# alexnodeland/fugue

Measured on AMD Instinct MI355X. Metric: hmc_leapfrog_steps_per_sec, higher is better.
Workload: dtype f64; 1 GPU; C2-normal32: hmc_chain, 32-site conjugate Normal (x#i~N(0,1), y#i~N(x#i,0.5)=0.2i-1), 65536 chains/GPU, L=16, HMCConfig::default; chains_per_gpu=65536, chains_total=65536, n_leapfrog=16, transitions_per_launch=25

## Files before the change

fugue_amd/csrc/fg_hmc_sep.hip:

```cpp
#include "fg_engine_internal.h"
#include "fg_gradstream.h"
#define FG_COLD_UKEY 1
#include "fg_cold.h"
#include "fg_hmc_sep_plan.h"

static_assert(FG_SEP_WAVE == FG_WAVE, "fg_hmc_sep_plan.h sizes tiles for 64-lane waves");

struct FgSepArgs {
    FgProgramDev P; FgChainCtx X; FgHmcDev H; FgSegSep seg;
    int iter0, n_steps, n_warmup, welford_on;
    double *draws; int first_sample_t;
    double *pos_all, *info;
};
static_assert(alignof(FgProgramDev) == 8 && alignof(FgChainCtx) == 8 && alignof(FgHmcDev) == 8 && alignof(FgSegSep) == 4, "kernarg layout of k_hmc_sep_steps");
static_assert(offsetof(FgSepArgs, X) == sizeof(FgProgramDev) && offsetof(FgSepArgs, H) == offsetof(FgSepArgs, X) + sizeof(FgChainCtx) &&
              offsetof(FgSepArgs, seg) == offsetof(FgSepArgs, H) + sizeof(FgHmcDev) && offsetof(FgSepArgs, iter0) == offsetof(FgSepArgs, seg) + sizeof(FgSegSep) &&
              offsetof(FgSepArgs, welford_on) == offsetof(FgSepArgs, iter0) + 12 && offsetof(FgSepArgs, draws) == ((offsetof(FgSepArgs, welford_on) + 4 + 7) & ~(size_t)7) &&
              offsetof(FgSepArgs, first_sample_t) == offsetof(FgSepArgs, draws) + 8 && offsetof(FgSepArgs, pos_all) == offsetof(FgSepArgs, draws) + 16 &&
              offsetof(FgSepArgs, info) == offsetof(FgSepArgs, draws) + 24, "kernarg layout of k_hmc_sep_steps: every argument at the next multiple of its alignment");

#ifdef FG_HMC_PROF
__device__ unsigned long long fg_hmc_prof[FG_SEP_WMAX][8];
#define FG_PROF_T(i) { const unsigned long long now_ = __builtin_readcyclecounter(); prof_[i] += now_ - tprev_; tprev_ = now_; }
#else
#define FG_PROF_T(i)
#endif
#ifndef FG_SEP_STAGGER
#define FG_SEP_STAGGER 2
#endif

__device__ __forceinline__ fg_u32x8 fg_sep_ld8(const FG_AS4 char *p) { return *(const FG_AS4 fg_u32x8 *)p; }
__device__ __forceinline__ fg_u32x4 fg_sep_ld4(const FG_AS4 char *p) { return *(const FG_AS4 fg_u32x4 *)p; }
__device__ __forceinline__ fg_u32x8 fg_sep_ld8(const char *p) { return *(const fg_u32x8 *)p; }
__device__ __forceinline__ fg_u32x4 fg_sep_ld4(const char *p) { return *(const fg_u32x4 *)p; }
__device__ __forceinline__ const FG_AS4 FgSepArgs *fg_sep_kernargs() {
    const FG_AS4 FgSepArgs *ka = (const FG_AS4 FgSepArgs *)__builtin_amdgcn_kernarg_segment_ptr();
    asm volatile("" : "+s"(ka));
    return ka;
}
__device__ __forceinline__ int fg_sep_scalar(int v) { asm volatile("" : "+s"(v)); return v; }
#define FG_SEP_LOAD(k) \
    const fg_u32x8 a##k = fg_sep_ld8(rb + 64 * k); \
    const fg_u32x4 b##k = fg_sep_ld4(rb + 64 * k + 32);

#define FG_SEP_Z(k, dl) (P2 ? (dl) * fg_dbl(a##k[4], a##k[5])                                                                   \
                            : ((a##k[0] & FG_G_POW2) ? (dl) * fg_dbl(a##k[4], a##k[5])                                           \
                                                     : ((a##k[0] & FG_G_DIV) ? (dl) / fg_dbl(b##k[0], b##k[1])                    \
                                                                             : fg_div_const((dl), fg_dbl(b##k[0], b##k[1]), fg_dbl(a##k[4], a##k[5])))))
#define FG_SEP_LP(k, z) (-0.5 * (z) * (z) - fg_dbl(a##k[6], a##k[7]) - 0.5 * FG_LN_2PI)
#define FG_SEP_DUAL(k, outp, outm)                                                                     \
    double outp, outm;                                                                                 \
    { const double c = fg_dbl(a##k[2], a##k[3]); const double zp = FG_SEP_Z(k, qp - c), zm = FG_SEP_Z(k, qm - c); \
      outp = FG_SEP_LP(k, zp); outm = FG_SEP_LP(k, zm); }
#define FG_SEP_NAN_NEG_INF(z, lp) { if (__builtin_expect(__any((z) != (z)), 0)) lp = ((z) != (z)) ? FG_NEG_INF : lp; }
#define FG_SEP_TERM_TO(k, dst)                                                                         \
    { const double z = FG_SEP_Z(k, q - fg_dbl(a##k[2], a##k[3])); double lp = FG_SEP_LP(k, z);       \
      FG_SEP_NAN_NEG_INF(z, lp) (dst)[a##k[1] * tw] = lp; }
#define FG_SEP_TERM(k) FG_SEP_TERM_TO(k, terms)
#define FG_SEP_LP_U(z) (-0.5 * (z) * (z) - 0.5 * FG_LN_2PI)
#define FG_SEP_LPF(k, z) (__builtin_fma(-0.5, (z) * (z), -fg_dbl(a##k[6], a##k[7])) - 0.5 * FG_LN_2PI)
#define FG_SEP_LPF_U(z) __builtin_fma(-0.5, (z) * (z), -0.5 * FG_LN_2PI)
#define FG_SEP_DUALF(k, outp, outm)                                                                    \
    double outp, outm;                                                                                 \
    { const double c = fg_dbl(a##k[2], a##k[3]); const double zp = FG_SEP_Z(k, qp - c), zm = FG_SEP_Z(k, qm - c); \
      outp = FG_SEP_LPF(k, zp); outm = FG_SEP_LPF(k, zm); }
#define FG_SEP_DUALS(k, outp, outm)                                                                    \
    double outp, outm;                                                                                 \
    { const double c = fg_dbl(a##k[2], a##k[3]); const double dp = qp - c, dm = qm - c;                \
      outp = __builtin_fma(nhs2_##k, dp * dp, -fg_dbl(a##k[6], a##k[7])) - 0.5 * FG_LN_2PI;            \
      outm = __builtin_fma(nhs2_##k, dm * dm, -fg_dbl(a##k[6], a##k[7])) - 0.5 * FG_LN_2PI; }
#define FG_SEPD_OWN(k, outp, outm) double outp, outm;                                                  \
    { const double c_ = fg_dbl(a##k[2], a##k[3]); const double zp_ = FG_SEP_Z(k, qp - c_), zm_ = FG_SEP_Z(k, qm - c_); \
      const double lp_ = FG_SEP_LP(k, zp_), lm_ = FG_SEP_LP(k, zm_);                                    \
      outp = (zp_ != zp_) ? FG_NEG_INF : lp_; outm = (zm_ != zm_) ? FG_NEG_INF : lm_; }

template <typename RB> struct FgSepScalarRb { static constexpr bool value = false; };
template <> struct FgSepScalarRb<const FG_AS4 char *> { static constexpr bool value = true; };

template <int NOBS, bool P2, bool CHECK, bool AN = false, bool U0 = false, bool FOLD = false, typename RB = const FG_AS4 char *, bool RANGED = false>
__device__ __forceinline__ bool fg_sep_trajectory(RB rb, double &q_io, double &p_io, double emi, double hk, int L, double h, double two_h,
                                                  double rcp_2h, double *terms, int tw, int nobs_rt, double c_hi = 0.0, double c_lo = 0.0) {
#define FG_SEP_HAS(k) (NOBS >= 0 ? NOBS >= (k) : nobs_rt >= (k))
    FG_SEP_LOAD(0) FG_SEP_LOAD(1) FG_SEP_LOAD(2) FG_SEP_LOAD(3)
    double q = q_io, p = p_io;
    bool bad = false;
    constexpr bool FOLDED = FOLD && P2 && !CHECK && !AN;
    double nhs2_0 = 0.0, nhs2_1 = 0.0, nhs2_2 = 0.0, nhs2_3 = 0.0;
#define FG_SEP_NHS2(k) if (FOLDED && (k > 0 || !U0) && FG_SEP_HAS(k)) { nhs2_##k = fg_dbl(b##k[2], b##k[3]); asm volatile("" : "+v"(nhs2_##k)); }
    FG_SEP_NHS2(0) FG_SEP_NHS2(1) FG_SEP_NHS2(2) FG_SEP_NHS2(3)
#undef FG_SEP_NHS2
    if (FOLD && !CHECK && !AN && FgSepScalarRb<RB>::value) asm volatile("" : "+s"(h), "+s"(c_hi), "+s"(c_lo));
    if (CHECK && !AN && NOBS >= 0 && FgSepScalarRb<RB>::value) asm volatile("" : "+s"(h));
    uint32_t nrange = 0u;
    auto grad = [&]() __attribute__((always_inline)) -> double {
        double g;
        if (AN) {
#define FG_SEP_ANTERM(k) { const double dl = q - fg_dbl(a##k[2], a##k[3]);                                                   \
        const double w = (P2 || (a##k[0] & FG_G_POW2)) ? (dl * fg_dbl(a##k[4], a##k[5])) * fg_dbl(a##k[4], a##k[5])         \
                                                       : (dl / fg_dbl(b##k[0], b##k[1])) / fg_dbl(b##k[0], b##k[1]); g = g - w; }
            g = 0.0;
            FG_SEP_ANTERM(0)
            if (FG_SEP_HAS(1)) FG_SEP_ANTERM(1)
            if (FG_SEP_HAS(2)) FG_SEP_ANTERM(2)
            if (FG_SEP_HAS(3)) FG_SEP_ANTERM(3)
#undef FG_SEP_ANTERM
        } else {
        const double qp = q + h, qm = q - h;
        double tp, tm;
        if (FOLDED) {
            if (U0) { tp = FG_SEP_LPF_U(qp); tm = FG_SEP_LPF_U(qm); }
            else { FG_SEP_DUALS(0, tp_, tm_) tp = tp_; tm = tm_; }
            if (FG_SEP_HAS(1)) {
                FG_SEP_DUALS(1, lp1, lm1)
                double sp = lp1, sm = lm1;
                if (FG_SEP_HAS(2)) { FG_SEP_DUALS(2, lp2, lm2) sp += lp2; sm += lm2; }
                if (FG_SEP_HAS(3)) { FG_SEP_DUALS(3, lp3, lm3) sp += lp3; sm += lm3; }
                tp = tp + sp; tm = tm + sm;
            }
        } else if (!CHECK) {
            if (U0) { tp = FG_SEP_LPF_U(qp); tm = FG_SEP_LPF_U(qm); }
            else { FG_SEP_DUALF(0, tp_, tm_) tp = tp_; tm = tm_; }
            if (FG_SEP_HAS(1)) {
                FG_SEP_DUALF(1, lp1, lm1)
                double sp = lp1, sm = lm1;
                if (FG_SEP_HAS(2)) { FG_SEP_DUALF(2, lp2, lm2) sp += lp2; sm += lm2; }
                if (FG_SEP_HAS(3)) { FG_SEP_DUALF(3, lp3, lm3) sp += lp3; sm += lm3; }
                tp = tp + sp; tm = tm + sm;
            }
        } else {
        if (U0) { tp = FG_SEP_LP_U(qp); tm = FG_SEP_LP_U(qm); }
        else { FG_SEP_DUAL(0, tp_, tm_) tp = tp_; tm = tm_; }
        if (FG_SEP_HAS(1)) {
            FG_SEP_DUAL(1, lp1, lm1)
            double sp = lp1, sm = lm1;
            if (FG_SEP_HAS(2)) { FG_SEP_DUAL(2, lp2, lm2) sp += lp2; sm += lm2; }
            if (FG_SEP_HAS(3)) { FG_SEP_DUAL(3, lp3, lm3) sp += lp3; sm += lm3; }
            tp = tp + sp; tm = tm + sm;
        }
        }
        const double n = tp - tm;
        if (!CHECK && FOLD) g = __builtin_fma(n, c_hi, n * c_lo);
        else g = fg_div_const(n, two_h, rcp_2h);
        if (!CHECK && FOLD && RANGED) {
        } else if (!CHECK && FOLD) {
            uint32_t hi = (uint32_t)__double2hiint(n);
            asm("" : "+v"(hi));
            const uint32_t nr = (hi << 1) - 0x19000000u;
            nrange = nrange > nr ? nrange : nr;
        } else {
        const double an = __builtin_fabs(n);
        if (__builtin_expect(__any(!(an >= 0x1p-823 && an <= 0x1p953)), 0)) g = n / two_h;
        }
        }
        if (CHECK) bad = bad || !fg_finite(g);
        return g;
    };
    { const double kick = hk * grad(); p = p + kick; asm volatile(""); q = q + emi * p; }
    for (int gs = 1; gs < L; ++gs) {
        const double kick = hk * grad();
        p = p + kick;
        asm volatile(""); p = p + kick;
        asm volatile(""); q = q + emi * p;
    }
    { const double kick = hk * grad(); p = p + kick; }
    if (!CHECK && FOLD && !RANGED && nrange >= 0xde000000u) p = __builtin_nan("");
    if (U0) { double lp = FG_SEP_LP_U(q); FG_SEP_NAN_NEG_INF(q, lp) terms[a0[1] * tw] = lp; }
    else FG_SEP_TERM(0)
    if (FG_SEP_HAS(1)) FG_SEP_TERM(1)
    if (FG_SEP_HAS(2)) FG_SEP_TERM(2)
    if (FG_SEP_HAS(3)) FG_SEP_TERM(3)
    q_io = q; p_io = p;
    return bad;
#undef FG_SEP_HAS
}

template <bool AN, typename RB>
__device__ __noinline__ FgD3 fg_sep_trajectory_checked(RB rb, double q, double p, double emi, double hk, int L, double h,
                                                       double two_h, double rcp_2h, double *terms, int tw, int nobs) {
    const bool bad = fg_sep_trajectory<-1, false, true, AN, false, false, RB>(rb, q, p, emi, hk, L, h, two_h, rcp_2h, terms, tw, nobs);
    FgD3 r; r.a = q; r.b = p; r.c = bad ? 1.0 : 0.0;
    return r;
}

template <int K, bool PSON>
__device__ __forceinline__ void fg_dense_add_rows(const double *p, int cnt, int tw, double &PS, double (&ap)[4], double (&am)[4]) {
#define FG_DENSE_BLOCK(R) { double y[R];                                                        \
        _Pragma("unroll") for (int q = 0; q < R; ++q) y[q] = p[q * tw];                         \
        _Pragma("unroll") for (int q = 0; q < R; ++q) { if (PSON) PS += y[q];                   \
            _Pragma("unroll") for (int jj = 0; jj < K; ++jj) { ap[jj] += y[q]; am[jj] += y[q]; } } \
        p += (long long)R * tw; }
    for (; cnt >= 8; cnt -= 8) FG_DENSE_BLOCK(8)
    if (cnt & 4) FG_DENSE_BLOCK(4)
    if (cnt & 2) FG_DENSE_BLOCK(2)
    if (cnt & 1) FG_DENSE_BLOCK(1)
#undef FG_DENSE_BLOCK
}
template <int NC>
__device__ __forceinline__ void fg_dense_section(const double *T, int tw, int lo, int hi, const int (&r)[4], const double (&tp)[4], const double (&tm)[4],
                                                 double (&ap)[4], double (&am)[4]) {
    double PS = 0.0;
    int pos = lo;
#define FG_DENSE_STEP(J) if (NC > J) {                                                          \
        fg_dense_add_rows<J, true>(T + (long long)pos * tw, r[J] - pos, tw, PS, ap, am);       \
        const double x = T[(long long)r[J] * tw];                                               \
        ap[J] = PS + tp[J]; am[J] = PS + tm[J];                                                 \
        _Pragma("unroll") for (int jj = 0; jj < J; ++jj) { ap[jj] += x; am[jj] += x; }          \
        if (NC > J + 1) PS += x;                                                                \
        pos = r[J] + 1; }
    FG_DENSE_STEP(0) FG_DENSE_STEP(1) FG_DENSE_STEP(2) FG_DENSE_STEP(3)
#undef FG_DENSE_STEP
    fg_dense_add_rows<NC, false>(T + (long long)pos * tw, hi - pos, tw, PS, ap, am);
}

template <int NC, bool OBS, bool MASS>
__device__ __forceinline__ bool fg_dense_trajectory(const FgProgramDev &P, const FgChainCtx &X, const FgHmcDev &H, const int (&own)[4], double *T0, double *T1,
                                                    double *kin0, double *kin1, int tw, int n_pri, int n_s, int L, double e, double h, double two_h,
                                                    double rcp_2h, uint32_t sk0, uint32_t sk1, uint32_t gchain, uint32_t iter, long long c, bool live) {
    int ci[4] = {0, 0, 0, 0}, rP[4] = {0, 0, 0, 0}, rO[4] = {0, 0, 0, 0};
    double q[4], p[4], k0v[4], mii[4], cP[4], sP[4], lP[4], cO[4], sO[4], lO[4];
    const double hk = 0.5 * e;
    const int blk_a = own[0] >> 1;
    int blk_b = blk_a;
#pragma unroll
    for (int j = 1; j < NC; ++j) if ((own[j] >> 1) != blk_a) blk_b = own[j] >> 1;
    const FgD2 za = fg_cold_normal_pair(sk0, sk1, gchain, (uint32_t)blk_a, iter, FG_RNG_HMC);
    FgD2 zb2 = za;
    if (NC > 2) zb2 = fg_cold_normal_pair(sk0, sk1, gchain, (uint32_t)blk_b, iter, FG_RNG_HMC);
#pragma unroll
    for (int j = 0; j < NC; ++j) {
        ci[j] = own[j];
        const FgSepCoord cd = P.sep_coord[ci[j]];
        const FG_AS4 char *rb = (const FG_AS4 char *)(uintptr_t)(P.sep + cd.off);
        { FG_SEP_LOAD(0) rP[j] = (int)a0[1]; cP[j] = fg_dbl(a0[2], a0[3]); sP[j] = fg_dbl(a0[4], a0[5]); lP[j] = fg_dbl(a0[6], a0[7]); (void)b0; }
        if (OBS) { FG_SEP_LOAD(1) rO[j] = (int)a1[1]; cO[j] = fg_dbl(a1[2], a1[3]); sO[j] = fg_dbl(a1[4], a1[5]); lO[j] = fg_dbl(a1[6], a1[7]); (void)b1; }
        const bool in_a = (ci[j] >> 1) == blk_a, second = (ci[j] & 1) != 0;
        const double z = in_a ? (second ? za.b : za.a) : (second ? zb2.b : zb2.a);
        mii[j] = MASS ? H.m_inv[(long long)ci[j] * X.C + c] : 1.0;
        p[j] = MASS ? z * H.mass_sqrt[(long long)ci[j] * X.C + c] : z;
        k0v[j] = MASS ? p[j] * p[j] * mii[j] : p[j] * p[j];
        q[j] = fg_as_double(X.values[(long long)P.f64_site[ci[j]] * X.C + c]);
    }
    bool bad = false;
    for (int gs = 0; gs <= L; ++gs) {
        double *T = ((L - gs) & 1) ? T1 : T0;
        double tpP[4], tmP[4], tpO[4], tmO[4];
#define FG_DENSE_LP(x_, c_, s_, l_, out) { const double z_ = ((x_) - (c_)) * (s_); const double lp_ = -0.5 * z_ * z_ - (l_) - 0.5 * FG_LN_2PI; \
                                           out = lp_; if (__builtin_expect(__any(z_ != z_), 0)) out = (z_ != z_) ? FG_NEG_INF : lp_; }
#pragma unroll
        for (int j = 0; j < NC; ++j) {
            const double qp = q[j] + h, qm = q[j] - h;
            double t0; FG_DENSE_LP(q[j], cP[j], sP[j], lP[j], t0) T[(long long)rP[j] * tw] = t0;
            FG_DENSE_LP(qp, cP[j], sP[j], lP[j], tpP[j]) FG_DENSE_LP(qm, cP[j], sP[j], lP[j], tmP[j])
            if (OBS) {
                double t1; FG_DENSE_LP(q[j], cO[j], sO[j], lO[j], t1) T[(long long)rO[j] * tw] = t1;
                FG_DENSE_LP(qp, cO[j], sO[j], lO[j], tpO[j]) FG_DENSE_LP(qm, cO[j], sO[j], lO[j], tmO[j])
            }
        }
#undef FG_DENSE_LP
        __syncthreads();
        double Pp[4], Pm[4], Lp[4], Lm[4];
        fg_dense_section<NC>(T, tw, 0, n_pri, rP, tpP, tmP, Pp, Pm);
        if (OBS) fg_dense_section<NC>(T, tw, n_pri, n_s, rO, tpO, tmO, Lp, Lm);
        else {
            double LS = 0.0;
            fg_dense_add_rows<0, true>(T + (long long)n_pri * tw, n_s - n_pri, tw, LS, Lp, Lm);
#pragma unroll
            for (int j = 0; j < NC; ++j) { Lp[j] = LS; Lm[j] = LS; }
        }
#pragma unroll
        for (int j = 0; j < NC; ++j) {
            const double n = (Pp[j] + Lp[j] + 0.0) - (Pm[j] + Lm[j] + 0.0);
            double g = fg_div_const(n, two_h, rcp_2h);
            const uint32_t ne = (uint32_t)(__double_as_longlong(n) >> 32) & 0x7fffffffu;
            if (__builtin_expect(__any(!((ne - 0x0c800000u) < 0x6f000000u)), 0)) g = n / two_h;
            bad = bad || !fg_finite(g);
            double pj = p[j] + hk * g;
            if (gs > 0 && gs < L) pj = pj + hk * g;
            p[j] = pj;
            if (gs < L) q[j] = q[j] + (MASS ? e * mii[j] : e) * pj;
        }
    }
#pragma unroll
    for (int j = 0; j < NC; ++j) {
        if (live) H.p0_scratch[(long long)ci[j] * X.C + c] = q[j];
        kin0[(long long)ci[j] * tw] = k0v[j];
        kin1[(long long)ci[j] * tw] = MASS ? p[j] * p[j] * mii[j] : p[j] * p[j];
    }
    return bad;
}

template <bool MASS, int MODE, int HALF = 0 , int NC = 0, int NOBS_R = 0, bool U0_R = false, bool FOLD = false,
          bool RANGED = false >
__global__ __launch_bounds__(FG_WAVE * FG_SEP_WMAX, 4) void k_hmc_sep_steps(FgProgramDev P, FgChainCtx X, FgHmcDev H, FgSegSep seg, int iter0, int n_steps,
                                                                             int n_warmup, int welford_on, double *draws, int first_sample_t,
                                                                             double *pos_all , double *info ) {
    extern __shared__ double lds[];
    constexpr int tw = FG_WAVE >> HALF;
    constexpr bool DFAST = MODE == 3, DENSE = MODE == 1 || DFAST, AN = MODE == 2;
    static_assert(!HALF || MODE == 0, "half tiles: sparse finite difference only");
    constexpr bool RES = NC > 0;
    constexpr int NCX = RES ? NC : 1;
    static_assert(!RES || (MODE == 0 && HALF == 0 && NC <= 4 && NOBS_R >= 0 && NOBS_R <= 3), "resident form: sparse 64-chain tiles");
    static_assert(!FOLD || MODE == 0, "the folded trajectory loop: sparse finite difference only");
    static_assert(!RANGED || FOLD, "the range test is the folded loop's");
    const int lane = threadIdx.x & (tw - 1);
    const int half = HALF == 1 ? (int)((threadIdx.x >> 5) & 1u) : (HALF == 2 ? (int)((threadIdx.x >> 4) & 3u) : 0);
    const int wv = __builtin_amdgcn_readfirstlane((int)(threadIdx.x >> 6));
    const long long chain = (long long)blockIdx.x * tw + lane;
    const bool live = chain < X.C;
    const bool live0 = live && half == 0;
    const long long c = live ? chain : X.C - 1;
    const int d = P.d, L = H.L, n_s = P.n_sstream, n_pri = P.n_prior_terms;
    const int srows = RES ? 0 : (P.n_sep_free > 0 ? P.n_slots : 0);
    double *slots = lds + lane;
    double *terms = lds + (long long)(srows + (DENSE ? 0 : 2 * d)) * tw + lane;
    double *xch = terms + (long long)n_s * tw;
    double *qrow = xch + 3 * tw, *prow = qrow + (long long)d * tw;
    double *kin0 = DENSE ? qrow : lds + (long long)srows * tw + lane;
    double *kin1 = DENSE ? prow : kin0 + (long long)d * tw;
    const int k0 = seg.c[wv], k1 = seg.c[wv + 1];
    const bool prio_turns = seg.c[FG_SEP_WMAX] == -1;
    const int stagger = seg.c[FG_SEP_WMAX] <= -2 ? -seg.c[FG_SEP_WMAX] - 1 : 0;
    const double *mi = MASS ? H.m_inv + c : nullptr;
    const double *ms = MASS ? H.mass_sqrt + c : nullptr;
    const double h = fg_uniform(H.h), two_h = FOLD ? 0.0 : fg_uniform(2.0 * H.h), rcp_2h = FOLD ? 0.0 : fg_uniform(1.0 / (2.0 * H.h));
    const double c_hi = H.div2_hi, c_lo = H.div2_lo;
#define FG_SEP_2H(th, rc) double th = two_h, rc = rcp_2h; if (FOLD) { double hh_ = h; asm volatile("" : "+v"(hh_)); th = 2.0 * hh_; rc = 1.0 / th; }
    const uint32_t sk0 = (uint32_t)X.seed, sk1 = (uint32_t)(X.seed >> 32), gchain = X.chain0 + (uint32_t)c;
    const int nown = k1 - k0;
    double qc[NCX], qpr[NCX], mir[NCX], msr[NCX];
    uint32_t roff[NCX];
    if (RES) {
#pragma unroll
        for (int j = 0; j < NCX; ++j) {
            const int i = j < nown ? k0 + j : 0;
            roff[j] = P.sep_coord[i].off;
            qc[j] = fg_as_double(X.values[(long long)P.f64_site[i] * X.C + c]);
            qpr[j] = qc[j];
            mir[j] = MASS ? H.m_inv[(long long)i * X.C + c] : 1.0;
            msr[j] = MASS ? H.mass_sqrt[(long long)i * X.C + c] : 1.0;
        }
    }
    double lj = 0.0, eps = 0.0, frozen = 0.0, da_mu = 0.0, da_leb = 0.0, da_hbar = 0.0, asum = 0.0, e_cur = 0.0;
    unsigned long long da_m = 0, ndiv = 0;
    if (wv == 0) {
        if (srows) fg_load_values(P, X, c, slots, tw);
        lj = H.lj[c]; eps = H.eps[c]; frozen = H.frozen[c];
        da_mu = H.da_mu[c]; da_leb = H.da_leb[c]; da_hbar = H.da_hbar[c]; da_m = H.da_m[c];
        for (int k = 0; k < P.n_sep_free; ++k) {
            const FgSepFree f = P.sep_free[k];
            const fg_u32x16 r = fg_fetch_grec(P.sstream, (int)f.sidx);
            FgAcc3 dummy = {0.0, 0.0, 0.0};
            terms[f.trow * tw] = fg_score_one<0>(r, slots[r[0] * tw], slots[r[1] * tw], P.pool, slots, tw, dummy);
        }
        if (iter0 < n_warmup) e_cur = eps;
        else {
            if (frozen == frozen) e_cur = frozen;
            else if (n_warmup > 0) e_cur = fg_cold_exp(da_leb);
            else e_cur = eps;
            frozen = e_cur;
        }
        xch[0] = e_cur;
        xch[2 * tw] = 0.0;
    }
    __syncthreads();
#ifdef FG_HMC_PROF
    unsigned long long prof_[8] = {0, 0, 0, 0, 0, 0, 0, 0}, tprev_ = __builtin_readcyclecounter();
#endif
    if (stagger && (stagger == 1 ? blockIdx.x >= (gridDim.x + 1) / 2 : (blockIdx.x & 1u) != 0u))
        for (int q = 0; q < FG_SEP_STAGGER; ++q) __builtin_amdgcn_s_sleep(64);
    FgD2 zpre = {0.0, 0.0};
    FgD2 zn[RES ? (NC + 1) / 2 : 1];
    bool have_pre = false;
    const uint32_t first_block = DENSE ? 0u : (HALF == 2 ? (uint32_t)(((k0 + half < d) ? k0 + half : k0) >> 1)
                                                         : (uint32_t)(k0 >> 1) + ((HALF == 1 && half && k0 + 2 < k1) ? 1u : 0u));
    for (int t = 0; t < n_steps; ++t) {
        const int iter = iter0 + t;
        const bool warming = iter < n_warmup;
        const double e = xch[0], hk = 0.5 * e;
        bool bad = false;
        double zb = 0.0;
        FgD2 zzh = {0.0, 0.0}; bool zh_next = false;
        const double *termsE = terms;
        int lnl = lane;
        long long cl = c;
        if (RES) { asm volatile("" : "+v"(lnl)); asm volatile("" : "+v"(cl)); }
        int prio_now = prio_turns ? -1 : 0;
        if constexpr (RES) {
            const FG_AS4 FgSepArgs *ka = fg_sep_kernargs();
            const double h = ka->H.h, c_hi = ka->H.div2_hi, c_lo = ka->H.div2_lo;
            const int L = ka->H.L, d = ka->P.d;
            prio_now = ka->seg.c[FG_SEP_WMAX];
            const FgSepRec *sep = ka->P.sep;
            const unsigned long long seed = ka->X.seed;
            const uint32_t sk0 = (uint32_t)seed, sk1 = (uint32_t)(seed >> 32), iter = (uint32_t)(ka->iter0 + t);
            const int pre = fg_sep_scalar((wv != 0 && t > 0) ? ka->seg.predraw : 0);
            const int nown_a = fg_sep_scalar(nown), k0_a = fg_sep_scalar(k0), turn = fg_sep_scalar((wv >> 2) & 1);
            double *termsR = lds + (long long)(2 * d) * tw + lnl;
            double *kin0R = lds + (long long)k0_a * tw + lnl;
            double *kin1R = kin0R + (long long)d * tw;
#pragma unroll
            for (int j = 0; j < NCX; ++j) {
                if (j >= nown_a) break;
                if (fg_sep_scalar(prio_now) == -1) { if ((j ^ turn) & 1) __builtin_amdgcn_s_setprio(1); else __builtin_amdgcn_s_setprio(0); }
                double z;
                if (!(j & 1)) { const FgD2 zz = pre ? zn[j >> 1] : fg_cold_normal_pair(sk0, sk1, gchain, (uint32_t)((k0_a + j) >> 1), iter, FG_RNG_HMC); z = zz.a; zb = zz.b; }
                else z = zb;
                double p = MASS ? z * msr[j] : z;
                const double mii = mir[j];
                kin0R[j * tw] = MASS ? p * p * mii : p * p;
                double q = qc[j];
                const double emi = MASS ? e * mii : e;
                const double q0 = q, p0 = p;
                const FG_AS4 char *rb = (const FG_AS4 char *)(uintptr_t)(sep + roff[j]);
                const int Lj = fg_sep_scalar(L);
                fg_sep_trajectory<NOBS_R, true, false, false, U0_R, FOLD, const FG_AS4 char *, RANGED>(rb, q, p, emi, hk, Lj, h, two_h, rcp_2h, termsR, tw, NOBS_R, c_hi, c_lo);
                if (__builtin_expect(__any(!fg_finite(p)), 0)) {
                    q = q0; p = p0;
                    FG_SEP_2H(th, rc)
                    bad = fg_sep_trajectory<NOBS_R, true, true, false, U0_R>(rb, q, p, emi, hk, Lj, h, th, rc, termsR, tw, NOBS_R) || bad;
                }
                qpr[j] = q;
                kin1R[j * tw] = MASS ? p * p * mii : p * p;
            }
        } else if (DFAST) {
            const int own[4] = { seg.own[wv][0], seg.own[wv][1], seg.own[wv][2], seg.own[wv][3] };
#define FG_DENSE_CALL(NC_, OBS_) fg_dense_trajectory<NC_, OBS_, MASS>(P, X, H, own, terms, qrow, kin0, kin1, tw, n_pri, n_s, L, e, h, two_h, rcp_2h, sk0, sk1, gchain, (uint32_t)iter, c, live)
            const int nown = seg.n_own[wv];
            if (n_s > n_pri) { if (nown == 4) bad = FG_DENSE_CALL(4, true); else if (nown == 3) bad = FG_DENSE_CALL(3, true); else if (nown == 2) bad = FG_DENSE_CALL(2, true); else bad = FG_DENSE_CALL(1, true); }
            else { if (nown == 4) bad = FG_DENSE_CALL(4, false); else if (nown == 3) bad = FG_DENSE_CALL(3, false); else if (nown == 2) bad = FG_DENSE_CALL(2, false); else bad = FG_DENSE_CALL(1, false); }
#undef FG_DENSE_CALL
        } else if (DENSE) {
            for (int i = k0; i < k1; ++i) {
                double z;
                if (!(i & 1)) { const FgD2 zz = fg_cold_normal_pair(sk0, sk1, gchain, (uint32_t)(i >> 1), (uint32_t)iter, FG_RNG_HMC); z = zz.a; zb = zz.b; }
                else z = zb;
                const double p = MASS ? z * ms[(long long)i * X.C] : z;
                prow[i * tw] = p;
                qrow[i * tw] = fg_as_double(X.values[(long long)P.f64_site[i] * X.C + c]);
            }
            for (int gs = 0; gs <= L; ++gs) {
                double *T = terms;
                if (gs > 0) __syncthreads();
                for (int i = k0; i < k1; ++i) {
                    const FgSepCoord cd = P.sep_coord[i];
                    const FG_AS4 char *rb = (const FG_AS4 char *)(uintptr_t)(P.sep + cd.off);
                    const int nobs = (cd.n & 7) - 1;
                    constexpr bool P2 = false;
                    FG_SEP_LOAD(0) FG_SEP_LOAD(1) FG_SEP_LOAD(2) FG_SEP_LOAD(3)
                    const double q = qrow[i * tw];
                    FG_SEP_TERM_TO(0, T)
                    if (nobs >= 1) FG_SEP_TERM_TO(1, T)
                    if (nobs >= 2) FG_SEP_TERM_TO(2, T)
                    if (nobs >= 3) FG_SEP_TERM_TO(3, T)
                }
                __syncthreads();
                int ppos = 0, lpos = n_pri;
                double PS = 0.0, LS = 0.0;
                for (int i = k0; i < k1; ++i) {
                    const FgSepCoord cd = P.sep_coord[i];
                    const FG_AS4 char *rb = (const FG_AS4 char *)(uintptr_t)(P.sep + cd.off);
                    const int nobs = (cd.n & 7) - 1;
                    constexpr bool P2 = false;
                    FG_SEP_LOAD(0) FG_SEP_LOAD(1) FG_SEP_LOAD(2) FG_SEP_LOAD(3)
                    const double q = qrow[i * tw];
                    const double qp = q + h, qm = q - h;
                    double Pp, Pm, Lp, Lm;
                    {
                        FG_SEPD_OWN(0, tp0, tm0)
                        const int r0 = (int)a0[1];
                        if (r0 < ppos) { ppos = 0; PS = 0.0; }
                        fg_inorder_run1<8>(T + (long long)ppos * tw, r0 - ppos, tw, PS);
                        ppos = r0;
                        Pp = PS + tp0; Pm = PS + tm0;
                        fg_inorder_run2<8>(T + (long long)(r0 + 1) * tw, n_pri - r0 - 1, tw, Pp, Pm);
                    }
                    {
                        int k = n_pri;
                        if (nobs >= 1) {
                            FG_SEPD_OWN(1, tp1, tm1)
                            const int r1 = (int)a1[1];
                            if (r1 < lpos) { lpos = n_pri; LS = 0.0; }
                            fg_inorder_run1<8>(T + (long long)lpos * tw, r1 - lpos, tw, LS);
                            lpos = r1;
                            Lp = LS + tp1; Lm = LS + tm1; k = r1 + 1;
                        } else { Lp = 0.0; Lm = 0.0; }
                        if (nobs >= 2) { FG_SEPD_OWN(2, tp2, tm2) const int r2 = (int)a2[1]; fg_inorder_run2<8>(T + (long long)k * tw, r2 - k, tw, Lp, Lm); Lp += tp2; Lm += tm2; k = r2 + 1; }
                        if (nobs >= 3) { FG_SEPD_OWN(3, tp3, tm3) const int r3 = (int)a3[1]; fg_inorder_run2<8>(T + (long long)k * tw, r3 - k, tw, Lp, Lm); Lp += tp3; Lm += tm3; k = r3 + 1; }
                        fg_inorder_run2<8>(T + (long long)k * tw, n_s - k, tw, Lp, Lm);
                    }
                    const double n = (Pp + Lp + 0.0) - (Pm + Lm + 0.0);
                    double g = fg_div_const(n, two_h, rcp_2h);
                    const uint32_t ne = (uint32_t)(__double_as_longlong(n) >> 32) & 0x7fffffffu;
                    if (__builtin_expect(__any(!((ne - 0x0c800000u) < 0x6f000000u)), 0)) g = n / two_h;
                    bad = bad || !fg_finite(g);
                    const double mii = MASS ? mi[(long long)i * X.C] : 1.0;
                    double p = prow[i * tw] + hk * g;
                    if (gs > 0 && gs < L) p = p + hk * g;
                    prow[i * tw] = p;
                    if (gs < L) qrow[i * tw] = q + (MASS ? e * mii : e) * p;
                }
            }
            termsE = terms;
            for (int i = k0; i < k1; ++i) {
                double z;
                if (!(i & 1)) { const FgD2 zz = fg_cold_normal_pair(sk0, sk1, gchain, (uint32_t)(i >> 1), (uint32_t)iter, FG_RNG_HMC); z = zz.a; zb = zz.b; }
                else z = zb;
                const double p0 = MASS ? z * ms[(long long)i * X.C] : z;
                const double mii = MASS ? mi[(long long)i * X.C] : 1.0;
                const double p = prow[i * tw];
                if (live) H.p0_scratch[(long long)i * X.C + c] = qrow[i * tw];
                kin0[i * tw] = MASS ? p0 * p0 * mii : p0 * p0;
                kin1[i * tw] = MASS ? p * p * mii : p * p;
            }
        } else
        for (int i = k0; i < k1; i += 1 << HALF) {
            if (prio_turns) { if (((i - k0) ^ (wv >> 2)) & 1) __builtin_amdgcn_s_setprio(1); else __builtin_amdgcn_s_setprio(0); }
            const bool on = !HALF || i + half < d;
            const int ci = HALF ? (on ? i + half : i) : i;
            double z;
            if (HALF == 2) {
                const FgD2 zz = (HALF != 0 && i == k0 && have_pre) ? zpre : fg_cold_normal_pair(sk0, sk1, gchain, (uint32_t)(ci >> 1), (uint32_t)iter, FG_RNG_HMC);
                z = (ci & 1) ? zz.b : zz.a;
            } else if (HALF) {
                if (!(((i - k0) >> 1) & 1)) {
                    zh_next = i + 2 < k1;
                    zzh = (HALF != 0 && i == k0 && have_pre) ? zpre : fg_cold_normal_pair(sk0, sk1, gchain, (uint32_t)(i >> 1) + ((half && zh_next) ? 1u : 0u), (uint32_t)iter, FG_RNG_HMC);
                    const double ob = __shfl_xor(zzh.b, 32, 64);
                    z = half ? (on ? (zh_next ? ob : zzh.b) : zzh.a) : zzh.a;
                } else {
                    const double oa = __shfl_xor(zzh.a, 32, 64);
                    z = half ? (on ? zzh.b : zzh.a) : oa;
                }
            }
            else if (!(i & 1)) { const FgD2 zz = (HALF != 0 && i == k0 && have_pre) ? zpre : fg_cold_normal_pair(sk0, sk1, gchain, (uint32_t)(i >> 1), (uint32_t)iter, FG_RNG_HMC); z = zz.a; zb = zz.b; }
            else z = zb;
            double p = MASS ? z * ms[(long long)ci * X.C] : z;
            const double mii = MASS ? mi[(long long)ci * X.C] : 1.0;
            if (on) kin0[ci * tw] = MASS ? p * p * mii : p * p;
            const long long gq = (long long)P.f64_site[ci] * X.C + c;
            double q = fg_as_double(X.values[gq]);
            const double emi = MASS ? e * mii : e;
            const FgSepCoord cd = P.sep_coord[i];
            const int nobs = (cd.n & 7) - 1;
            const double q0 = q, p0 = p;
            if (HALF) {
                const char *rb = (const char *)(P.sep + P.sep_coord[ci].off);
#define FG_SEP_CALLH(NO, UU) fg_sep_trajectory<NO, true, false, false, UU, FOLD, const char *, RANGED>(rb, q, p, emi, hk, L, h, two_h, rcp_2h, terms, tw, NO, c_hi, c_lo)
                if ((cd.n & 512) && nobs == 1) FG_SEP_CALLH(1, true);
                else if (nobs == 1) FG_SEP_CALLH(1, false); else if (nobs == 0) FG_SEP_CALLH(0, false); else if (nobs == 2) FG_SEP_CALLH(2, false); else FG_SEP_CALLH(3, false);
#undef FG_SEP_CALLH
                if (__builtin_expect(__any(!fg_finite(p)), 0)) {
                    FG_SEP_2H(th, rc)
                    const FgD3 r = fg_sep_trajectory_checked<AN, const char *>(rb, q0, p0, emi, hk, L, h, th, rc, terms, tw, nobs);
                    q = r.a; p = r.b; bad = bad || (on && r.c != 0.0);
                }
            } else {
            const FG_AS4 char *rb = (const FG_AS4 char *)(uintptr_t)(P.sep + cd.off);
#define FG_SEP_CALL(NO, PP) fg_sep_trajectory<NO, PP, false, AN, false, FOLD, const FG_AS4 char *, RANGED>(rb, q, p, emi, hk, L, h, two_h, rcp_2h, terms, tw, NO, c_hi, c_lo)
            if (!AN && (cd.n & 512) && nobs == 1) fg_sep_trajectory<1, true, false, false, true, FOLD, const FG_AS4 char *, RANGED>(rb, q, p, emi, hk, L, h, two_h, rcp_2h, terms, tw, 1, c_hi, c_lo);
            else if (cd.n & 256) { if (nobs == 1) FG_SEP_CALL(1, true); else if (nobs == 0) FG_SEP_CALL(0, true); else if (nobs == 2) FG_SEP_CALL(2, true); else FG_SEP_CALL(3, true); }
            else { if (nobs == 1) FG_SEP_CALL(1, false); else if (nobs == 0) FG_SEP_CALL(0, false); else if (nobs == 2) FG_SEP_CALL(2, false); else FG_SEP_CALL(3, false); }
#undef FG_SEP_CALL
            if (__builtin_expect(__any(!fg_finite(p)), 0)) {
                FG_SEP_2H(th, rc)
                const FgD3 r = fg_sep_trajectory_checked<AN, const FG_AS4 char *>(rb, q0, p0, emi, hk, L, h, th, rc, terms, tw, nobs);
                q = r.a; p = r.b; bad = bad || r.c != 0.0;
            }
            }
            if (live && on) H.p0_scratch[(long long)ci * X.C + c] = q;
            if (on) kin1[ci * tw] = MASS ? p * p * mii : p * p;
        }
        if (bad) atomicOr((unsigned long long *)(xch + 2 * tw), 1ull);
        if (prio_now == -1) { if (wv == 0) __builtin_amdgcn_s_setprio(2); else __builtin_amdgcn_s_setprio(0); }
        FG_PROF_T(0)
        __syncthreads();
        FG_PROF_T(1)
#define FG_SEP_ARG(kp, field, plain) (RES ? (kp)->field : (plain))
        const FG_AS4 FgSepArgs *kb = RES ? fg_sep_kernargs() : nullptr;
        const int d_b = FG_SEP_ARG(kb, P.d, d), n_pri_b = FG_SEP_ARG(kb, P.n_prior_terms, n_pri), n_s_b = FG_SEP_ARG(kb, P.n_sstream, n_s);
        const int n_steps_b = FG_SEP_ARG(kb, n_steps, n_steps), n_warmup_b = FG_SEP_ARG(kb, n_warmup, n_warmup), iter_b = RES ? kb->iter0 + t : iter;
        const uint32_t sk0_b = RES ? (uint32_t)kb->X.seed : sk0, sk1_b = RES ? (uint32_t)(kb->X.seed >> 32) : sk1;
        const int prio_b = FG_SEP_ARG(kb, seg.c[FG_SEP_WMAX], prio_now);
        const int W = (int)(blockDim.x >> 6);
        const bool sum4_plain = HALF != 0 && seg.sum4 != 0 && W >= 4;
        const int sum4_w = RES ? kb->seg.sum4 * W : 0;
#define FG_SEP_S(x) (RES ? fg_sep_scalar(x) : (x))
#define FG_SEP_SUM4 (RES ? fg_sep_scalar(sum4_w) >= 4 : sum4_plain)
        double s0 = 0.0;
        if (FG_SEP_SUM4) {
            if (wv == 0) s0 = fg_inorder_sum1(kin0, d_b, tw);
            else if (wv == 1) xch[3 * tw] = fg_inorder_sum1(kin1, d_b, tw);
            else if (wv == 2) xch[4 * tw] = fg_inorder_sum1(termsE, n_pri_b, tw);
            else if (wv == 3) xch[5 * tw] = fg_inorder_sum1(termsE + (long long)n_pri_b * tw, n_s_b - n_pri_b, tw);
            if (wv == (W > 4 ? 4 : 3)) xch[6 * tw] = fg_cold_u01_pair(sk0_b, sk1_b, gchain, (uint32_t)((d_b + 1) >> 1), (uint32_t)iter_b, FG_RNG_HMC).a;
            __syncthreads();
        }
        have_pre = false;
        if constexpr (RES) {
            if (fg_sep_scalar((wv != 0 && t + 1 < n_steps_b) ? kb->seg.predraw : 0)) {
                const int nown_b = fg_sep_scalar(nown);
#pragma unroll
                for (int jp = 0; jp < (NCX + 1) / 2; ++jp)
                    if (2 * jp < nown_b) zn[jp] = fg_cold_normal_pair(sk0_b, sk1_b, gchain, (uint32_t)(k0 >> 1) + (uint32_t)jp, (uint32_t)(iter_b + 1), FG_RNG_HMC);
            }
        }
        if (HALF != 0 && seg.sum4 != 0 && wv != 0 && t + 1 < n_steps && k0 < k1 && !(k0 & 1)) {
            zpre = fg_cold_normal_pair(sk0, sk1, gchain, first_block, (uint32_t)(iter + 1), FG_RNG_HMC);
            have_pre = true;
        }
        if (wv == 0) {
            double s1, pri, lik;
            if (FG_SEP_SUM4) { s1 = xch[3 * tw]; pri = xch[4 * tw]; lik = xch[5 * tw]; }
            else {
                fg_inorder_sums2<8>(kin0, d_b, kin1, d_b, tw, s0, s1);
                fg_inorder_sums2<8>(termsE, n_pri_b, termsE + (long long)n_pri_b * tw, n_s_b - n_pri_b, tw, pri, lik);
            }
            const double h0 = -lj + 0.5 * s0;
            const double lj_new = pri + lik + 0.0;
            bool div = fg_as_i64(xch[2 * tw]) != 0;
            div = div || !fg_finite(lj_new);
            double ap = 0.0; bool acc = false;
            if (!div) {
                const double h_new = -lj_new + 0.5 * s1;
                ap = fg_cold_accept_prob(h0, h_new);
                const double u = FG_SEP_SUM4 ? xch[6 * tw] : fg_cold_u01_pair(sk0_b, sk1_b, gchain, (uint32_t)((d_b + 1) >> 1), (uint32_t)iter_b, FG_RNG_HMC).a;
                acc = u < ap;
            }
            if (acc) lj = lj_new;
            xch[tw] = acc ? 1.0 : 0.0;
            asum += ap; ndiv += div ? 1ull : 0ull;
            double *const info_b = FG_SEP_ARG(kb, info, info);
            if (live0 && info_b) {
                const long long C_b = FG_SEP_ARG(kb, X.C, X.C);
                double *r = info_b + (long long)t * 4 * C_b + c;
                r[0] = acc ? 1.0 : 0.0; r[C_b] = div ? 1.0 : 0.0; r[2 * C_b] = ap; r[3 * C_b] = e_cur;
            }
            if (iter_b < n_warmup_b) {
                da_m += 1ull;
                const FgD3 r = fg_cold_da_update(da_hbar, da_leb, (double)da_m, da_mu, FG_SEP_ARG(kb, H.target, H.target), ap);
                eps = r.a; da_hbar = r.b; da_leb = r.c;
            }
            if (iter_b + 1 < n_warmup_b) e_cur = eps;
            else {
                if (frozen == frozen) e_cur = frozen;
                else if (n_warmup_b > 0) e_cur = fg_cold_exp(da_leb);
                else e_cur = eps;
                if (t + 1 < n_steps_b) frozen = e_cur;
            }
            if (t + 1 < n_steps_b) xch[0] = e_cur;
            xch[2 * tw] = 0.0;
        }
        FG_PROF_T(2)
        if (prio_b == -1) __builtin_amdgcn_s_setprio(0);
        __syncthreads();
        FG_PROF_T(3)
        const FG_AS4 FgSepArgs *kc = RES ? fg_sep_kernargs() : nullptr;
        const long long C_c = FG_SEP_ARG(kc, X.C, X.C);
        const int d_c = FG_SEP_ARG(kc, P.d, d), first_c = FG_SEP_ARG(kc, first_sample_t, first_sample_t);
        double *const draws_c = FG_SEP_ARG(kc, draws, draws), *const pos_c = FG_SEP_ARG(kc, pos_all, pos_all);
        const int left_c = RES ? kc->n_warmup - (kc->iter0 + t) : 0, welf_c = FG_SEP_ARG(kc, welford_on, welford_on);
#define FG_SEP_WARM_C (RES ? fg_sep_scalar(left_c) > 0 : warming)
        const bool acc = xch[tw] != 0.0;
        unsigned long long wn = 0;
        double wnd = 0.0;
        if (FG_SEP_WARM_C && FG_SEP_S(welf_c)) {
            wn = FG_SEP_ARG(kc, H.w_n, H.w_n)[c] + 1ull;
            wnd = (double)wn;
            asm volatile("" : "+v"(wnd));
        }
        auto commit = [&](int i, double x, bool on, long long cc) {
            if (live && on && pos_c) pos_c[((long long)t * d_c + i) * C_c + cc] = x;
            if (FG_SEP_WARM_C) {
                if (FG_SEP_S(welf_c)) {
                    double *const w_mean = FG_SEP_ARG(kc, H.w_mean, H.w_mean), *const w_m2 = FG_SEP_ARG(kc, H.w_m2, H.w_m2);
                    const long long gi = (long long)i * C_c + cc;
                    const double n = wnd;
                    double mean = w_mean[gi];
                    const double delta = x - mean;
                    mean += delta / n;
                    const double delta2 = x - mean;
                    if (live && on) { w_mean[gi] = mean; w_m2[gi] += delta * delta2; }
                }
            } else if (draws_c && live && on) draws_c[((long long)(t - first_c) * d_c + i) * C_c + cc] = x;
        };
        if (RES) {
            const int nown_c = fg_sep_scalar(nown), k0_c = fg_sep_scalar(k0);
#pragma unroll
            for (int j = 0; j < NCX; ++j) {
                if (j >= nown_c) break;
                const double x = acc ? qpr[j] : qc[j];
                qc[j] = x;
                commit(k0_c + j, x, true, cl);
            }
        } else
        for (int jo = 0; jo < (DFAST ? seg.n_own[wv] : k1 - k0); jo += 1 << HALF) {
            const int i0 = DFAST ? seg.own[wv][jo] : k0 + jo;
            const bool on = !HALF || i0 + half < d;
            const int i = HALF ? (on ? i0 + half : i0) : i0;
            const long long g = (long long)P.f64_site[i] * X.C + c;
            const double x = acc ? H.p0_scratch[(long long)i * X.C + c] : fg_as_double(X.values[g]);
            if (acc && live && on) X.values[g] = fg_as_i64(x);
            commit(i, x, on, c);
        }
        if (FG_SEP_WARM_C && FG_SEP_S(welf_c)) {
            __syncthreads();
            if (wv == 0 && live0) FG_SEP_ARG(kc, H.w_n, H.w_n)[c] = wn;
        }
        FG_PROF_T(4)
    }
#undef FG_SEP_ARG
#undef FG_SEP_S
#undef FG_SEP_SUM4
#undef FG_SEP_WARM_C
#ifdef FG_HMC_PROF
    if (blockIdx.x == 0 && lane == 0) for (int q = 0; q < 8; ++q) fg_hmc_prof[wv][q] = prof_[q];
#endif
    const FG_AS4 FgSepArgs *ke = RES ? fg_sep_kernargs() : nullptr;
    if (RES && live) {
#pragma unroll
        for (int j = 0; j < NCX; ++j)
            if (j < nown) ke->X.values[(long long)ke->P.f64_site[k0 + j] * ke->X.C + c] = fg_as_i64(qc[j]);
    }
    if (wv == 0 && live0) {
        const FgHmcDev &Hs = RES ? *(const FgHmcDev *)&ke->H : H;
        Hs.lj[c] = lj; Hs.eps[c] = eps; Hs.frozen[c] = frozen;
        Hs.da_mu[c] = da_mu; Hs.da_leb[c] = da_leb; Hs.da_hbar[c] = da_hbar; Hs.da_m[c] = da_m;
        Hs.alpha_sum[c] += asum; Hs.n_div[c] += ndiv;
    }
}

using FgSepKernel = void (*)(FgProgramDev, FgChainCtx, FgHmcDev, FgSegSep, int, int, int, int, double *, int, double *, double *);
struct FgSepVariant { FgSepKey key; FgSepKernel fn, fn_ranged; unsigned long long raised, raised_ranged; };
template <bool M, int MODE, int HALF, int NC, int NOBS, bool U0, bool FOLD> static constexpr FgSepKernel fg_sep_ranged_fn() {
    if constexpr (FOLD && !(M && HALF == 0 && NC == 0)) return k_hmc_sep_steps<M, MODE, HALF, NC, NOBS, U0, true, true>; else return nullptr;
}
#define FG_SEP_ENTRY(M, MODE, HALF, NC, NOBS, U0, FOLD) { { M, MODE, HALF, NC, NOBS, U0, FOLD }, k_hmc_sep_steps<M, MODE, HALF, NC, NOBS, U0, FOLD>, fg_sep_ranged_fn<M, MODE, HALF, NC, NOBS, U0, FOLD>(), 0, 0 },
static FgSepVariant fg_sep_variants[] = { FG_SEP_VARIANTS(FG_SEP_ENTRY) };
#undef FG_SEP_ENTRY

int fg_hmc_sep_launch(fg_engine *e, int iter0, int n, int welford_on, double *draws, int first_sample_t, double *pos_all, double *info) {
    if (!fg_hmc_sep_gate(e->gt, e->P.sep != nullptr, e->sep_disabled, e->d)) return FG_E_UNSUPPORTED;
    const FgSepPlanIn in = { e->C, e->d, e->n_simd, e->n_slots, e->P.n_sep_free, e->P.n_sstream, e->cfg.grad_mode, e->H.use_mass != 0, e->mw_override,
                             e->gt, e->sep_disabled, e->sep_res_disabled, e->sep_fold_disabled, e->prog->sep_fold && e->H.div2 != 0 , &e->prog->sep_coord, &e->prog->sep,
                             fg_env_switch("FG_HMC_SEP_HALF"), fg_env_switch("FG_HMC_DENSE_FAST"), fg_env_switch("FG_HMC_SUM4"), fg_env_switch("FG_HMC_PRIO"),
                             fg_env_switch("FG_HMC_STAGGER"), fg_env_switch("FG_HMC_PREDRAW") };
    FgSepPlan pl;
    int rc = fg_hmc_sep_plan(in, &pl);
    if (rc != FG_OK) return rc;
    FgSepVariant *v = std::find_if(std::begin(fg_sep_variants), std::end(fg_sep_variants), [&](const FgSepVariant &q) { return q.key == pl.key; });
    if (v == std::end(fg_sep_variants)) return FG_E_UNSUPPORTED;
    const bool ranged = v->fn_ranged && e->H.range != 0 && !fg_switch_is(fg_env_switch("FG_HMC_SEP_RANGE"), 0);
    rc = fg_launch(e, ranged ? v->fn_ranged : v->fn, ranged ? v->raised_ranged : v->raised, dim3(pl.tiles), dim3(FG_WAVE * pl.W), pl.lds, e->P, e->X, e->H, pl.seg, iter0, n, e->n_warmup, welford_on, draws, first_sample_t, pos_all, info);
    if (rc == FG_OK) e->last_hmc_kernel = pl.name;
    return rc;
}

#ifdef FG_HMC_PROF
extern "C" int fg_debug_hmc_prof(unsigned long long *out) {
    return hipMemcpyFromSymbol(out, HIP_SYMBOL(fg_hmc_prof), sizeof(unsigned long long) * FG_SEP_WMAX * 8) == hipSuccess ? 0 : -1;
}
#endif
```

Measured before the change: 31.03 billion leapfrog-steps/s.

## Carry the final leapfrog gradient across HMC transitions to skip the first gradient

Caches the gradient computed at the end of each trajectory in registers and reuses it as the first half-kick gradient of the next transition when the proposal is accepted, keeping the old one on rejection. An initial gradient is computed once per launch before the loop. This removes one of L+1 gradient evaluations per trajectory, at the cost of extra per-site registers, and it is disabled for configurations expected to hit register pressure (NC=4 with mass or unfolded 3 observations).

```diff
diff --git a/fugue_amd/csrc/fg_hmc_sep.hip b/fugue_amd/csrc/fg_hmc_sep.hip
--- a/fugue_amd/csrc/fg_hmc_sep.hip
+++ b/fugue_amd/csrc/fg_hmc_sep.hip
@@ -77,9 +77,9 @@
 template <typename RB> struct FgSepScalarRb { static constexpr bool value = false; };
 template <> struct FgSepScalarRb<const FG_AS4 char *> { static constexpr bool value = true; };
 
-template <int NOBS, bool P2, bool CHECK, bool AN = false, bool U0 = false, bool FOLD = false, typename RB = const FG_AS4 char *, bool RANGED = false>
+template <int NOBS, bool P2, bool CHECK, bool AN = false, bool U0 = false, bool FOLD = false, typename RB = const FG_AS4 char *, bool RANGED = false, int CARRY = 0>
 __device__ __forceinline__ bool fg_sep_trajectory(RB rb, double &q_io, double &p_io, double emi, double hk, int L, double h, double two_h,
-                                                  double rcp_2h, double *terms, int tw, int nobs_rt, double c_hi = 0.0, double c_lo = 0.0) {
+                                                  double rcp_2h, double *terms, int tw, int nobs_rt, double c_hi = 0.0, double c_lo = 0.0, double *g_io = nullptr) {
 #define FG_SEP_HAS(k) (NOBS >= 0 ? NOBS >= (k) : nobs_rt >= (k))
     FG_SEP_LOAD(0) FG_SEP_LOAD(1) FG_SEP_LOAD(2) FG_SEP_LOAD(3)
     double q = q_io, p = p_io;
@@ -155,14 +155,17 @@
         if (CHECK) bad = bad || !fg_finite(g);
         return g;
     };
-    { const double kick = hk * grad(); p = p + kick; asm volatile(""); q = q + emi * p; }
+    if constexpr (CARRY == 3) { *g_io = grad(); return bad; }
+    double g_first = 0.0;
+    if constexpr (CARRY == 1) g_first = *g_io; else g_first = grad();
+    { const double kick = hk * g_first; p = p + kick; asm volatile(""); q = q + emi * p; }
     for (int gs = 1; gs < L; ++gs) {
         const double kick = hk * grad();
         p = p + kick;
         asm volatile(""); p = p + kick;
         asm volatile(""); q = q + emi * p;
     }
-    { const double kick = hk * grad(); p = p + kick; }
+    { const double g_last = grad(); if constexpr (CARRY != 0) *g_io = g_last; const double kick = hk * g_last; p = p + kick; }
     if (!CHECK && FOLD && !RANGED && nrange >= 0xde000000u) p = __builtin_nan("");
     if (U0) { double lp = FG_SEP_LP_U(q); FG_SEP_NAN_NEG_INF(q, lp) terms[a0[1] * tw] = lp; }
     else FG_SEP_TERM(0)
@@ -289,6 +292,10 @@
     return bad;
 }
 
+constexpr bool fg_sep_carries(bool MASS, int NC, int NOBS, bool U0, bool FOLD, bool RANGED) {
+    (void)U0; (void)RANGED;
+    return NC > 0 && !(NC == 4 && (MASS || (NOBS == 3 && !FOLD)));
+}
 template <bool MASS, int MODE, int HALF = 0 , int NC = 0, int NOBS_R = 0, bool U0_R = false, bool FOLD = false,
           bool RANGED = false >
 __global__ __launch_bounds__(FG_WAVE * FG_SEP_WMAX, 4) void k_hmc_sep_steps(FgProgramDev P, FgChainCtx X, FgHmcDev H, FgSegSep seg, int iter0, int n_steps,
@@ -341,6 +348,24 @@
             msr[j] = MASS ? H.mass_sqrt[(long long)i * X.C + c] : 1.0;
         }
     }
+    constexpr bool CARRIES = fg_sep_carries(MASS, NC, NOBS_R, U0_R, FOLD, RANGED);
+    constexpr int NCG = CARRIES ? NC : 1;
+    double gc[NCG], gpr[NCG];
+    if constexpr (CARRIES) {
+        const FG_AS4 FgSepArgs *kp = fg_sep_kernargs();
+        const double h = kp->H.h;
+        const FgSepRec *sep = kp->P.sep;
+        const int nown_p = fg_sep_scalar(nown);
+        FG_SEP_2H(th, rc)
+#pragma unroll
+        for (int j = 0; j < NCG; ++j) {
+            gc[j] = 0.0; gpr[j] = 0.0;
+            if (j >= nown_p) continue;
+            double q = qc[j], p = 0.0;
+            const FG_AS4 char *rb = (const FG_AS4 char *)(uintptr_t)(sep + roff[j]);
+            fg_sep_trajectory<NOBS_R, true, true, false, U0_R, false, const FG_AS4 char *, false, 3>(rb, q, p, 0.0, 0.0, 0, h, th, rc, nullptr, tw, NOBS_R, 0.0, 0.0, &gc[j]);
+        }
+    }
     double lj = 0.0, eps = 0.0, frozen = 0.0, da_mu = 0.0, da_leb = 0.0, da_hbar = 0.0, asum = 0.0, e_cur = 0.0;
     unsigned long long da_m = 0, ndiv = 0;
     if (wv == 0) {
@@ -414,12 +439,15 @@
                 const double q0 = q, p0 = p;
                 const FG_AS4 char *rb = (const FG_AS4 char *)(uintptr_t)(sep + roff[j]);
                 const int Lj = fg_sep_scalar(L);
-                fg_sep_trajectory<NOBS_R, true, false, false, U0_R, FOLD, const FG_AS4 char *, RANGED>(rb, q, p, emi, hk, Lj, h, two_h, rcp_2h, termsR, tw, NOBS_R, c_hi, c_lo);
+                double g = 0.0;
+                if constexpr (CARRIES) g = gc[j];
+                fg_sep_trajectory<NOBS_R, true, false, false, U0_R, FOLD, const FG_AS4 char *, RANGED, CARRIES ? 1 : 0>(rb, q, p, emi, hk, Lj, h, two_h, rcp_2h, termsR, tw, NOBS_R, c_hi, c_lo, &g);
                 if (__builtin_expect(__any(!fg_finite(p)), 0)) {
                     q = q0; p = p0;
                     FG_SEP_2H(th, rc)
-                    bad = fg_sep_trajectory<NOBS_R, true, true, false, U0_R>(rb, q, p, emi, hk, Lj, h, th, rc, termsR, tw, NOBS_R) || bad;
+                    bad = fg_sep_trajectory<NOBS_R, true, true, false, U0_R, false, const FG_AS4 char *, false, CARRIES ? 2 : 0>(rb, q, p, emi, hk, Lj, h, th, rc, termsR, tw, NOBS_R, 0.0, 0.0, &g) || bad;
                 }
+                if constexpr (CARRIES) gpr[j] = g;
                 qpr[j] = q;
                 kin1R[j * tw] = MASS ? p * p * mii : p * p;
             }
@@ -691,6 +719,7 @@
                 if (j >= nown_c) break;
                 const double x = acc ? qpr[j] : qc[j];
                 qc[j] = x;
+                if constexpr (CARRIES) gc[j] = acc ? gpr[j] : gc[j];
                 commit(k0_c + j, x, true, cl);
             }
         } else
```

Result: faster. 31.87 billion leapfrog-steps/s, median of 6 (+2.7%).
